# istellartech/GELATO

Hardware: NVIDIA B200
Metric: fd_jacobian_plus_residual_evals_per_s (higher is better)
Workload: dtype f64

## Files before the change

### gelato_b200/csrc/gelato_b200.cu

```cuda
#include <cuda_runtime.h>

#include <cstdio>
#include <cstdlib>
#include <cstring>
#include <string>
#include <thread>
#include <utility>
#include <vector>

#include "host_pool.h"
#include "plan_host.h"

#ifndef GJ_MIN_BLOCKS
#define GJ_MIN_BLOCKS 2
#endif
#ifndef GJ_PREFETCH_BLOCKS
#define GJ_PREFETCH_BLOCKS 296
#endif
__device__ __forceinline__ void prefetch_batch_l2(const double* x_all, size_t n_doubles, int blocks, int threads) {
#if GJ_PREFETCH_BLOCKS > 0
  if ((int)blockIdx.x < blocks) {
    const size_t lines = (n_doubles * sizeof(double) + 127) / 128;
    for (size_t l = (size_t)blockIdx.x * threads + threadIdx.x; l < lines; l += (size_t)blocks * threads)
      asm volatile("prefetch.global.L2 [%0];" ::"l"(reinterpret_cast<const char*>(x_all) + l * 128));
  }
#endif
}
#ifdef GJ_CLOCKS
__device__ unsigned long long gj_clk_sum[8][16][6];
#define GJ_CLK_DECL long long clk_[6] = {0, 0, 0, 0, 0, 0}
#define GJ_CLK(i) clk_[i] = clock64()
#define GJ_CLK_FLUSH(role, two)                                                                         \
  if ((threadIdx.x & 31) == 0) {                                                                        \
    unsigned long long* c = gj_clk_sum[(role) & 7][threadIdx.x >> 5];                                   \
    atomicAdd(c + 0, (unsigned long long)(clk_[1] - clk_[0]));                                              \
    atomicAdd(c + 1, (unsigned long long)(clk_[2] - clk_[1]));                                              \
    atomicAdd(c + 2, (unsigned long long)((two) ? 0 : clk_[3] - clk_[2]));                                  \
    atomicAdd(c + 3, (unsigned long long)((two) ? 0 : clk_[4] - clk_[3]));                                  \
    atomicAdd(c + 4, (unsigned long long)(clk_[5] - clk_[4]));                                              \
    atomicAdd(c + 5, 1ull);                                                                             \
  }
#else
#define GJ_CLK_DECL
#define GJ_CLK(i)
#define GJ_CLK_FLUSH(role, two)
#endif
template <int ROLES>
__device__ __forceinline__ void jacobian_body(const PlanView& P, const int32_t* __restrict__ block_table, const int n_scen,
                                              const int32_t* __restrict__ scen_ids, const double* __restrict__ x_all,
                                              double* __restrict__ out_all, double* __restrict__ g_all) {
  __shared__ JacStore store;
  const JacScratch sm = jac_scratch(store);
  prefetch_batch_l2(x_all, (size_t)n_scen * P.n_vars, GJ_PREFETCH_BLOCKS, GJ_THREADS);
  const int scen = blockIdx.x % n_scen;
  const int32_t* bt = block_table + (size_t)(blockIdx.x / n_scen) * BT_COLS;
  const double* x = x_all + (size_t)scen * P.n_vars;
  double* out = out_all + (size_t)scen * (size_t)(P.packed ? P.n_pack : P.n_vals);
  double* g = g_all ? g_all + (size_t)scen * P.n_rows : nullptr;
  const int sid = scen_ids ? scen_ids[scen] : scen;
  const bool two_phase = jac_role_two_phase(bt[BT_ROLE]);
  GJ_CLK_DECL;
  GJ_CLK(0);
  jac_block_phase<ROLES>(P, sid, bt, x, out, g, threadIdx.x, 0, sm);
  GJ_CLK(1);
  __syncthreads();
  GJ_CLK(2);
  if (!two_phase) {
    jac_block_phase<ROLES>(P, sid, bt, x, out, g, threadIdx.x, 2, sm);
    GJ_CLK(3);
    __syncthreads();
  }
  GJ_CLK(4);
  jac_block_phase<ROLES>(P, sid, bt, x, out, g, threadIdx.x, 3, sm);
  GJ_CLK(5);
  GJ_CLK_FLUSH(bt[BT_ROLE], two_phase);
}
__global__ void __launch_bounds__(GJ_THREADS, GJ_MIN_BLOCKS)
k_jacobian(const __grid_constant__ PlanView P, const int32_t* __restrict__ block_table, const int n_scen, const int32_t* __restrict__ scen_ids,
           const double* __restrict__ x_all, double* __restrict__ out_all, double* __restrict__ g_all) {
  jacobian_body<JR_ALL>(P, block_table, n_scen, scen_ids, x_all, out_all, g_all);
}
__global__ void __launch_bounds__(GJ_THREADS, GJ_MIN_BLOCKS)
k_jacobian_heavy(const __grid_constant__ PlanView P, const int32_t* __restrict__ block_table, const int n_scen,
                 const int32_t* __restrict__ scen_ids, const double* __restrict__ x_all, double* __restrict__ out_all,
                 double* __restrict__ g_all) {
  jacobian_body<JR_HEAVY>(P, block_table, n_scen, scen_ids, x_all, out_all, g_all);
}
__global__ void __launch_bounds__(GJ_THREADS, GJ_MIN_BLOCKS)
k_jacobian_light(const __grid_constant__ PlanView P, const int32_t* __restrict__ block_table, const int n_scen,
                 const int32_t* __restrict__ scen_ids, const double* __restrict__ x_all, double* __restrict__ out_all,
                 double* __restrict__ g_all) {
  jacobian_body<JR_LIGHT>(P, block_table, n_scen, scen_ids, x_all, out_all, g_all);
}

#define GV_THREADS (32 * GV_PARTS)
#ifndef GV_MIN_BLOCKS
#define GV_MIN_BLOCKS 5
#endif
__global__ void __launch_bounds__(GV_THREADS, GV_MIN_BLOCKS)
k_jacobian_noair(const __grid_constant__ PlanView P, const int first, const int count, const int n_scen,
                 const int32_t* __restrict__ scen_ids, const double* __restrict__ x_all, double* __restrict__ out_all,
                 double* __restrict__ g_all) {
  const int per = (count + 31) / 32;
  const int scen = blockIdx.x / per;
  const int lane = threadIdx.x & 31, part = threadIdx.x >> 5;
  const int k = (blockIdx.x - scen * per) * 32 + lane;
  __shared__ double grav[32][NPV * 3];
  const double* x = x_all + (size_t)scen * P.n_vars;
  double* out = out_all + (size_t)scen * (size_t)(P.packed ? P.n_pack : P.n_vals);
  double* g = g_all ? g_all + (size_t)scen * P.n_rows : nullptr;
  const int sid = scen_ids ? scen_ids[scen] : scen;
  const bool live = k < count;
  NodeRef nr;
  if (live) {
    nr = jac_node(P, first + k);
    for (int pv = part; pv < NPV; pv += GV_PARTS) dyn_noair_gravity(P, sid, x, nr, pv, grav[lane] + 3 * pv);
  }
  __syncthreads();
  if (live) dyn_noair_part(P, sid, x, out, g, nr, part, grav[lane]);
}

#ifndef GR_MIN_BLOCKS
#define GR_MIN_BLOCKS 8
#endif
__global__ void __launch_bounds__(GR_THREADS, GR_MIN_BLOCKS)
// ... 52 lines not shown
__global__ void k_fp64_muladd(double* out, int iters) {
  double a0 = threadIdx.x * 1e-9, a1 = a0 + 1, a2 = a0 + 2, a3 = a0 + 3, a4 = a0 + 4, a5 = a0 + 5, a6 = a0 + 6,
         a7 = a0 + 7;
  const double b = 1.0000001, c = 1e-9;
  for (int i = 0; i < iters; i++) {
    a0 = __dadd_rn(__dmul_rn(a0, b), c); a1 = __dadd_rn(__dmul_rn(a1, b), c);
    a2 = __dadd_rn(__dmul_rn(a2, b), c); a3 = __dadd_rn(__dmul_rn(a3, b), c);
    a4 = __dadd_rn(__dmul_rn(a4, b), c); a5 = __dadd_rn(__dmul_rn(a5, b), c);
    a6 = __dadd_rn(__dmul_rn(a6, b), c); a7 = __dadd_rn(__dmul_rn(a7, b), c);
  }
  out[blockIdx.x * blockDim.x + threadIdx.x] = a0 + a1 + a2 + a3 + a4 + a5 + a6 + a7;
}

static thread_local std::string g_err;
static int fail(int code, const std::string& msg) {
  g_err = msg;
  return code;
}
#define CU(call)                                                                                  \
  do {                                                                                            \
    cudaError_t e_ = (call);                                                                      \
    if (e_ != cudaSuccess)                                                                        \
      return fail(GELATO_ERR_CUDA, std::string(#call) + ": " + cudaGetErrorString(e_));           \
  } while (0)

struct GelatoPlan {
  int device = 0;
  PlanView view{};
  std::vector<void*> owned;
  int32_t* jac_blocks = nullptr;
  int n_jac_blocks = 0, n_jac_main = 0;
  int32_t *jac_heavy = nullptr, *jac_light = nullptr;
  int n_jac_heavy = 0, n_jac_light = 0;
  int vac_first = 0, n_vac = 0;
  int32_t* res_blocks = nullptr;
  int n_res_blocks = 0;
  long long n_pack = 0;
  std::vector<int64_t> pk_full, pk_src;
  std::vector<double> pk_sgn;
  std::vector<void*> scen_owned;
  double *d_packed = nullptr, *h_packed = nullptr;
  size_t cap_packed = 0;
  double *d_px = nullptr, *d_pg = nullptr, *h_px = nullptr;
  int32_t* d_pids = nullptr;
  bool pids_iota = false;
  size_t cap_px = 0;
  double* vals_template = nullptr;
  long long vals_template_sstride = 0;
  int n_scen_cfg = 1;
  cudaStream_t stream = nullptr;
  double *d_x = nullptr, *d_g = nullptr, *d_vals = nullptr;
  double *h_x = nullptr, *h_out = nullptr;
  size_t cap_scen = 0;
  cudaGraphExec_t res_graph = nullptr;
  int res_graph_n = 0;
  double* h_small_out = nullptr;
  size_t cap_small_out = 0;
  int32_t* d_ids = nullptr;
  double* d_vals_ids = nullptr;
  size_t cap_ids = 0;
  const int64_t* d_xdep = nullptr;
  std::vector<int64_t> h_xdep;
  long long n_xdep = 0;
  double *d_pack = nullptr, *h_pack = nullptr;
  size_t cap_pack = 0;
  int host_threads = 0;
// ... 26 lines not shown
  void* d = nullptr;
  CU(cudaMalloc(&d, count * sizeof(T)));
  p->owned.push_back(d);
  CU(cudaMemcpy(d, src, count * sizeof(T), cudaMemcpyHostToDevice));
  *dst = static_cast<const T*>(d);
  return GELATO_OK;
}

struct JacRange {
  int b0 = 0, nb = -1, v0 = 0, nv = 0;
};
static int launch_jacobian(GelatoPlan* p, const double* x_dev, double* out_dev, double* g_dev, int n_scen, cudaStream_t st,
                           cudaStream_t aux, cudaEvent_t ev_fork, cudaEvent_t ev_join, const int32_t* ids_dev, bool packed,
                           JacRange rg = JacRange()) {
  PlanView v = p->view;
  v.packed = packed ? 1 : 0;
  const bool all = rg.nb < 0;
  const int nb = all ? (g_dev ? p->n_jac_blocks : p->n_jac_main) : rg.nb;
  const int nv = all ? p->n_vac : rg.nv;
  const int v_first = p->vac_first + (all ? 0 : rg.v0);
  const int32_t* table = p->jac_blocks + (size_t)(all ? 0 : rg.b0) * BT_COLS;
  const bool side = nv > 0 && nb > 0 && aux != st;
  if (side) {
    CU(cudaEventRecord(ev_fork, st));
    CU(cudaStreamWaitEvent(aux, ev_fork, 0));
  }
  if (nv > 0) {
    const int per = (nv + 31) / 32;
    k_jacobian_noair<<<(unsigned)per * n_scen, GV_THREADS, 0, side ? aux : st>>>(v, v_first, nv, n_scen, ids_dev, x_dev, out_dev,
                                                                                g_dev);
    p->launches++;
  }
  if (nb > 0) {
    k_jacobian<<<(unsigned)nb * n_scen, GJ_THREADS, 0, st>>>(v, table, n_scen, ids_dev, x_dev, out_dev, g_dev);
    p->launches++;
  }
  CU(cudaGetLastError());
  if (side) {
    CU(cudaEventRecord(ev_join, aux));
    CU(cudaStreamWaitEvent(st, ev_join, 0));
  }
  return GELATO_OK;
}

extern "C" {

const char* gelato_last_error(void) { return g_err.c_str(); }
void gelato_set_error_(const char* msg) { g_err = msg ? msg : ""; }

int gelato_device_count(void) {
  int n = 0;
  if (cudaGetDeviceCount(&n) != cudaSuccess) return 0;
  return n;
}

int gelato_plan_create(const GelatoPlanDesc* d, int device, GelatoPlan** out) {
  if (!d || !out) return fail(GELATO_ERR_ARG, "null argument");
  if (const char* why = validate_desc(d)) return fail(GELATO_ERR_ARG, why);
  int ndev = 0;
  cudaError_t e = cudaGetDeviceCount(&ndev);
  if (e != cudaSuccess || ndev == 0)
    return fail(GELATO_ERR_CUDA, "no CUDA device: the B200 kernels are the only evaluation path (no CPU fallback)");
  CU(cudaSetDevice(device));
  GelatoPlan* p = new GelatoPlan();
  p->device = device;
  PlanView& v = p->view;
  planview_scalars(d, v);
// ... 25 lines not shown
    p->h_xdep.assign(d->xdep_idx, d->xdep_idx + d->n_xdep);
    p->n_xdep = d->n_xdep;
    const int64_t* dx = nullptr;
    if ((rc = upload(p, d->xdep_idx, (size_t)d->n_xdep, &dx)) != GELATO_OK) { gelato_plan_destroy(p); return rc; }
    p->d_xdep = dx;
    std::vector<int64_t> small;
    for (int64_t i = 0; i < d->n_xdep;) {
      int64_t j = i + 1;
      while (j < d->n_xdep && d->xdep_idx[j] == d->xdep_idx[j - 1] + 1) j++;
      if (j - i >= 512) p->big_runs.push_back({d->xdep_idx[i], j - i});
      else small.insert(small.end(), d->xdep_idx + i, d->xdep_idx + j);
      i = j;
    }
    p->n_small = (long long)small.size();
    p->h_small = small;
    if ((rc = upload(p, small.data(), small.size(), &dx)) != GELATO_OK) { gelato_plan_destroy(p); return rc; }
    p->d_xdep_small = dx;
  }
  const double* tmpl = nullptr;
  if ((rc = upload(p, d->vals_template, (size_t)d->n_vals, &tmpl)) != GELATO_OK) { gelato_plan_destroy(p); return rc; }
  p->vals_template = const_cast<double*>(tmpl);
#undef UP

  HostTables ht;
  build_host_tables(d, ht);
  const int32_t* tb = nullptr;
  p->n_jac_blocks = (int)(ht.jac_blocks.size() / BT_COLS);
  p->n_res_blocks = (int)(ht.res_blocks.size() / BT_COLS);
  p->n_jac_main = ht.n_jac_main;
  p->vac_first = ht.vac_first;
  p->n_vac = ht.n_vac;
  p->n_jac_heavy = (int)(ht.jac_heavy.size() / BT_COLS);
  p->n_jac_light = (int)(ht.jac_light.size() / BT_COLS);
  if ((rc = upload(p, ht.jac_heavy.data(), ht.jac_heavy.size(), &tb)) != GELATO_OK) { gelato_plan_destroy(p); return rc; }
  p->jac_heavy = const_cast<int32_t*>(tb);
  if ((rc = upload(p, ht.jac_light.data(), ht.jac_light.size(), &tb)) != GELATO_OK) { gelato_plan_destroy(p); return rc; }
  p->jac_light = const_cast<int32_t*>(tb);
  {
    PackedLayout L;
    build_packed_layout(d, L);
    if (d->xdep_idx && d->n_xdep > 0 &&
        ((size_t)d->n_xdep != L.full_slot.size() || !std::equal(L.full_slot.begin(), L.full_slot.end(), d->xdep_idx))) {
      gelato_plan_destroy(p);
      return fail(GELATO_ERR_ARG, "xdep_idx is not the set of slots the Jacobian kernel writes for this plan");
    }
    p->n_pack = L.n_pack;
    v.n_pack = L.n_pack;
    if ((rc = upload(p, L.sec_pk.data(), L.sec_pk.size(), &v.sec_pk)) != GELATO_OK) { gelato_plan_destroy(p); return rc; }
    if ((rc = upload(p, L.aero_pk.data(), L.aero_pk.size(), &v.aero_pk)) != GELATO_OK) { gelato_plan_destroy(p); return rc; }
    if ((rc = upload(p, L.evt_pk.data(), L.evt_pk.size(), &v.evt_pk)) != GELATO_OK) { gelato_plan_destroy(p); return rc; }
    p->pk_full.swap(L.full_slot);
    p->pk_src.swap(L.src);
    p->pk_sgn.swap(L.sgn);
  }
  if ((rc = upload(p, ht.jac_blocks.data(), ht.jac_blocks.size(), &tb)) != GELATO_OK) { gelato_plan_destroy(p); return rc; }
  p->jac_blocks = const_cast<int32_t*>(tb);
  if ((rc = upload(p, ht.res_blocks.data(), ht.res_blocks.size(), &tb)) != GELATO_OK) { gelato_plan_destroy(p); return rc; }
  p->res_blocks = const_cast<int32_t*>(tb);
  if ((rc = upload(p, ht.node_rec.data(), ht.node_rec.size(), &v.node_rec)) != GELATO_OK) { gelato_plan_destroy(p); return rc; }
  if ((rc = upload(p, ht.jac_rec.data(), ht.jac_rec.size(), &v.jac_rec)) != GELATO_OK) { gelato_plan_destroy(p); return rc; }
  if ((rc = upload(p, ht.aero_rows.data(), ht.aero_rows.size(), &v.aero_rows)) != GELATO_OK) { gelato_plan_destroy(p); return rc; }
  v.n_aero_rows = (int)ht.aero_rows.size();

  cudaError_t ce = cudaStreamCreateWithFlags(&p->stream, cudaStreamNonBlocking);
  if (ce == cudaSuccess) ce = cudaStreamCreateWithFlags(&p->copy_stream, cudaStreamNonBlocking);
  if (ce == cudaSuccess) ce = cudaEventCreateWithFlags(&p->ev_kernel, cudaEventDisableTiming);
// ... 739 lines not shown
    CU(cudaGetLastError());
    float ms = 0.f;
    CU(cudaEventElapsedTime(&ms, p->ev0, p->ev1));
    out_ms[piece] = ms / reps;
  }
  return GELATO_OK;
}

int gelato_host_alloc(size_t bytes, void** out) {
  if (!out) return fail(GELATO_ERR_ARG, "null");
  CU(cudaMallocHost(out, bytes));
  return GELATO_OK;
}

int gelato_host_free(void* ptr) {
  if (ptr) CU(cudaFreeHost(ptr));
  return GELATO_OK;
}

int gelato_launch_kernel_dev(GelatoPlan* p, int which, const double* x_dev, double* out_dev, double* g_dev, int32_t n_scen,
                             int32_t packed, void* stream) {
  int rc = check_scen(p, n_scen);
  if (rc) return rc;
  CU(cudaSetDevice(p->device));
  cudaStream_t st = stream ? (cudaStream_t)stream : p->stream;
  PlanView v = p->view;
  v.packed = packed ? 1 : 0;
  if (which == 0) {
    k_residuals<<<(unsigned)p->n_res_blocks * n_scen, GR_THREADS, 0, st>>>(v, p->res_blocks, n_scen, nullptr, x_dev, out_dev);
  } else if (which == 1) {
    return launch_jacobian(p, x_dev, out_dev, g_dev, n_scen, st, p->pair_stream, p->ev_fork, p->ev_join, nullptr, packed != 0);
  } else if (which == 2) {
    if (p->n_jac_heavy == 0) return fail(GELATO_ERR_ARG, "the plan has no heavy blocks");
    k_jacobian_heavy<<<(unsigned)p->n_jac_heavy * n_scen, GJ_THREADS, 0, st>>>(v, p->jac_heavy, n_scen, nullptr, x_dev, out_dev, g_dev);
  } else if (which == 3) {
    if (p->n_jac_light == 0) return fail(GELATO_ERR_ARG, "the plan has no light blocks");
    k_jacobian_light<<<(unsigned)p->n_jac_light * n_scen, GJ_THREADS, 0, st>>>(v, p->jac_light, n_scen, nullptr, x_dev, out_dev, g_dev);
  } else if (which == 5) {
    if (p->n_vac == 0) return fail(GELATO_ERR_ARG, "the plan has no vacuum nodes");
    const int per = (p->n_vac + 31) / 32;
    k_jacobian_noair<<<(unsigned)per * n_scen, GV_THREADS, 0, st>>>(v, p->vac_first, p->n_vac, n_scen, nullptr, x_dev, out_dev, g_dev);
  } else if (which == 6) {
    const int nb = g_dev ? p->n_jac_blocks : p->n_jac_main;
    if (nb == 0) return fail(GELATO_ERR_ARG, "the plan has no Jacobian blocks");
    k_jacobian<<<(unsigned)nb * n_scen, GJ_THREADS, 0, st>>>(v, p->jac_blocks, n_scen, nullptr, x_dev, out_dev, g_dev);
  } else {
    return fail(GELATO_ERR_ARG, "which must be 0, 1, 2, 3, 5 or 6");
  }
  p->launches++;
  CU(cudaGetLastError());
  return GELATO_OK;
}

int gelato_time_kernel(GelatoPlan* p, int which, const double* x_dev, double* out_dev, int32_t n_scen, int reps,
                       float* avg_ms) {
  int rc = check_scen(p, n_scen);
  if (rc) return rc;
  if (reps <= 0 || !avg_ms) return fail(GELATO_ERR_ARG, "bad reps");
  CU(cudaSetDevice(p->device));
  CU(cudaStreamSynchronize(p->stream));
  CU(cudaEventRecord(p->ev0, p->stream));
  for (int i = 0; i < reps; i++) {
    if (which == 0) {
      k_residuals<<<(unsigned)p->n_res_blocks * n_scen, GR_THREADS, 0, p->stream>>>(p->view, p->res_blocks, n_scen, nullptr, x_dev, out_dev);
    } else if (which == 1) {
      if ((rc = launch_jacobian(p, x_dev, out_dev, nullptr, n_scen, p->stream, p->pair_stream, p->ev_fork, p->ev_join, nullptr,
                                false)))
        return rc;
      continue;
    } else if (which == 2) {
      if (p->n_jac_heavy > 0)
        k_jacobian_heavy<<<(unsigned)p->n_jac_heavy * n_scen, GJ_THREADS, 0, p->stream>>>(p->view, p->jac_heavy, n_scen, nullptr,
                                                                                        x_dev, out_dev, nullptr);
    } else {
      if (p->n_jac_light > 0)
        k_jacobian_light<<<(unsigned)p->n_jac_light * n_scen, GJ_THREADS, 0, p->stream>>>(p->view, p->jac_light, n_scen, nullptr,
                                                                                        x_dev, out_dev, nullptr);
    }
    p->launches++;
  }
  CU(cudaEventRecord(p->ev1, p->stream));
  CU(cudaEventSynchronize(p->ev1));
  CU(cudaGetLastError());
  float ms = 0.f;
  CU(cudaEventElapsedTime(&ms, p->ev0, p->ev1));
  *avg_ms = ms / reps;
  return GELATO_OK;
}

int gelato_selftest_unfused(int device, int* ok) {
  if (!ok) return fail(GELATO_ERR_ARG, "null");
  CU(cudaSetDevice(device));
  double* d = nullptr;
  CU(cudaMalloc(&d, sizeof(double)));
  k_unfused_probe<<<1, 1>>>(1.0 + 0x1p-30, 1.0 - 0x1p-30, -1.0, d);
  double h = 1.0;
  CU(cudaMemcpy(&h, d, sizeof(double), cudaMemcpyDeviceToHost));
  cudaFree(d);
  *ok = (h == 0.0);
  return GELATO_OK;
}

int gelato_fp64_peak(int device, double* tflops_fma, double* tflops_nofma) {
  CU(cudaSetDevice(device));
  cudaDeviceProp prop;
  CU(cudaGetDeviceProperties(&prop, device));
  const int blocks = prop.multiProcessorCount * 8, threads = 256, iters = 1 << 14;
  double* d = nullptr;
  CU(cudaMalloc(&d, (size_t)blocks * threads * sizeof(double)));
  cudaEvent_t e0, e1;
// ... 39 lines not shown
```

### gelato_b200/csrc/jobs.h

```cpp
#ifndef GELATO_B200_JOBS_H_
#define GELATO_B200_JOBS_H_

#include "../../include/gelato_b200.h"
#include "physics.h"

#ifndef GJ_THREADS
#define GJ_THREADS 448
#endif
#ifndef GJ_NODES
#define GJ_NODES 32
#endif
#ifndef GD_NODES
#define GD_NODES 32
#endif
#ifndef GJ_A_THREADS
#define GJ_A_THREADS 160
#endif
#ifndef GJA_A_THREADS
#define GJA_A_THREADS 192
#endif
#ifndef GD_GRAVITY_IN_POS
#define GD_GRAVITY_IN_POS 0
#endif
#ifndef GN_NODES
// ... 3 lines not shown
#define GN_A_THREADS 160
#endif
#ifndef GJ_EVT_PER_WARP
#define GJ_EVT_PER_WARP 0
#endif
#ifndef GJ_EVT
#define GJ_EVT (GJ_THREADS / (GJ_EVT_PER_WARP ? 32 : 16))
#endif
#ifndef GG_NODES
#define GG_NODES (GJ_THREADS / 16)
#endif
#define GR_THREADS 128
#define GR_NODES 64
#define NPV 5
#define NRV 7
#define NPVA 6
#define NRVA 8
#define NQV 8

static_assert(GJ_A_THREADS % 32 == 0 && GJ_A_THREADS < GJ_THREADS && GJ_THREADS % 32 == 0, "phase-0 thread groups are whole warps");
static_assert(GJA_A_THREADS % 32 == 0 && GJA_A_THREADS < GJ_THREADS, "phase-0 thread groups are whole warps");
static_assert(GN_A_THREADS % 32 == 0 && GN_A_THREADS < GJ_THREADS, "no-air thread groups are whole warps");
static_assert(GG_NODES * 16 <= GJ_THREADS && GJ_EVT * 16 <= GJ_THREADS, "lane maps");
#define GJ_MAX2(a, b) ((a) > (b) ? (a) : (b))
#define GJ_FQ_NODES GJ_MAX2(GJ_MAX2(GN_NODES, GD_NODES), GG_NODES)
#define GJ_PR_NODES GJ_MAX2(GJ_NODES, GD_NODES)
static_assert(GJ_THREADS * 3 <= GJ_FQ_NODES * 14 * 3, "event jobs keep 3 values per thread in f");
static_assert(GN_NODES * NPV * 3 <= GJ_PR_NODES * NPVA * 8, "no-air gravity items fit the pp array");
static_assert(GR_THREADS == 2 * GR_NODES, "residual phase 0 uses two threads per node");

enum { BR_DYN_AIR = 0, BR_DYN_NOAIR, BR_DYN_GEN, BR_AERO, BR_EVT, BR_LIN, BR_DYN  };
enum { BT_ROLE = 0, BT_JOB, BT_START, BT_COUNT, BT_COLS };
#define GJ_PHASES 4

struct PlanView {
  int S, N, M, n_vars, n_rows;
  long long n_vals;
  int payload_mode;
  int off_pos, off_vel, off_quat, off_u, off_t;
  const int32_t* sec_i32;
  const int64_t* sec_i64;
  const double* sec_f64;
  long long sec_f64_sstride;
  const double* d_pool;
  const double* tau_pool;
  const double* wind;
  long long wind_sstride;
  int n_wind;
  const double* ca;
  int n_ca;
  Units un;
  const double* unit_mass_scen;
  int n_lin;
  const int32_t* lin_i32;
  const double* lin_f64;
  const double* lin_const_scen;
  int n_aero;
  const int32_t* aero_i32;
  const int64_t* aero_i64;
  const double* aero_f64;
  const uint8_t* rc_aero;
  int n_evt;
  const int32_t* evt_i32;
  const int64_t* evt_i64;
  const double* evt_f64;
  const struct NodeRec* node_rec;
// ... 959 lines not shown
    return;
  }
  if (type == GE_USER_ORBIT) {
    for (int r = 0; r < ei[GE_NROW]; r++)
      vals[ej[GE_J_POS] + r * GE_USER_AUX + (lane - 1)] = fd_div(sm.f[3 * tid + r] - sm.f[3 * c + r], dx);
    return;
  }
  const int comp = ei[GE_COMP], form = ei[GE_FORM];
  const double gfd = fd_div(sm.f[3 * tid + comp] - sm.f[3 * c + comp], dx);
  const double val = evt_form_grad(form, gfd, ef[GE_REF], ef[GE_DEN]);
  if (type == GE_IIP) {
    if (lane == 7) vals[ej[GE_J_T]] = val;
    else if (lane & 1) vals[ej[GE_J_POS] + (lane - 1) / 2] = val;
    else vals[ej[GE_J_VEL] + (lane - 2) / 2] = val;
  } else {
    if (lane == 4) vals[ej[GE_J_T]] = val;
    else vals[ej[GE_J_POS] + (lane - 1)] = val;
  }
}

P_HD void lin_res(const PlanView& P, int scen, const double* x, double* g, int k) {
  const int32_t* li = P.lin_i32 + k * GL_I32_COLS;
  const double* lf = P.lin_f64 + k * GL_F64_COLS;
  const double a = (li[GL_IDX_PLUS] >= 0) ? x[li[GL_IDX_PLUS]] * lf[GL_SCALE_PLUS] : 0.0;
  const double b = (li[GL_IDX_MINUS] >= 0) ? x[li[GL_IDX_MINUS]] * lf[GL_SCALE_MINUS] : 0.0;
  const double c = P.lin_const_scen ? P.lin_const_scen[(long long)scen * P.n_lin + k] : lf[GL_CONST];
  g[li[GL_ROW]] = (a - b) + c;
}

#define JR_HEAVY ((1 << BR_DYN_AIR) | (1 << BR_AERO))
#define JR_LIGHT ((1 << BR_DYN_NOAIR) | (1 << BR_DYN_GEN) | (1 << BR_EVT) | (1 << BR_LIN))
#define JR_ALL (JR_HEAVY | JR_LIGHT)
P_HD void lin_res(const PlanView& P, int scen, const double* x, double* g, int k);
template <int ROLES>
GM_HD_INL void jac_block_phase(const PlanView& P, int scen, const int32_t* bt, const double* x, double* vals, double* g,
                          int tid, int phase, const JacScratch& sm) {
  const int start = bt[BT_START], count = bt[BT_COUNT], role = bt[BT_ROLE];
  if ((ROLES >> BR_DYN_AIR & 1) && role == BR_DYN_AIR) dyn_air_phase(P, scen, x, vals, g, start, count, tid, phase, sm);
  if ((ROLES >> BR_AERO & 1) && role == BR_AERO) aero_phase(P, scen, x, vals, g, start, count, tid, phase, sm);
  if ((ROLES >> BR_DYN_NOAIR & 1) && role == BR_DYN_NOAIR) dyn_noair_phase(P, scen, x, vals, g, start, count, tid, phase, sm);
  if ((ROLES >> BR_DYN_GEN & 1) && role == BR_DYN_GEN) dyn_gen_phase(P, scen, x, vals, g, start, count, tid, phase, sm);
  if ((ROLES >> BR_EVT & 1) && role == BR_EVT && (tid >> (GJ_EVT_PER_WARP ? 5 : 4)) < count &&
      (!GJ_EVT_PER_WARP || (tid & 31) < 16)) {
    const int job = tid >> (GJ_EVT_PER_WARP ? 5 : 4);
    const int slot = job * 16 + (tid & (GJ_EVT_PER_WARP ? 31 : 15));
    if (phase == 0) evt_jac_phase1(P, scen, x, start + job, slot, g != nullptr, sm);
    else if (phase == 3) evt_jac_phase2(P, vals, g, start + job, slot, sm);
  }
  if ((ROLES >> BR_LIN & 1) && role == BR_LIN && phase == 3 && g) {
    if (tid < count) lin_res(P, scen, x, g, start + tid);
    if (start == 0 && tid == 0) g[0] = P.payload_mode ? -x[0] : x[P.off_t + P.S];
  }
}
P_HD bool jac_role_two_phase(int role) { return role == BR_EVT || role == BR_DYN_GEN || role == BR_LIN; }

P_HD void res_block_phase0(const PlanView& P, int scen, const int32_t* bt, const double* x, int tid, ResScratch& sm) {
  if (bt[BT_ROLE] == BR_DYN) dyn_res_phase0(P, scen, x, bt[BT_START], bt[BT_COUNT], tid, sm);
}
P_HD void res_block_phase1(const PlanView& P, int scen, const int32_t* bt, const double* x, double* g, int tid,
                           ResScratch& sm) {
  switch (bt[BT_ROLE]) {
    case BR_DYN: dyn_res_phase1(P, scen, x, bt[BT_START], bt[BT_COUNT], tid, sm); break;
    case BR_AERO:
      if (tid < bt[BT_COUNT]) {
        aero_res(P, scen, x, g, P.aero_rows[bt[BT_START] + tid]);
      }
      break;
    case BR_EVT:
      if (tid < bt[BT_COUNT]) evt_res(P, scen, x, g, bt[BT_START] + tid);
      break;
    case BR_LIN:
      if (tid < bt[BT_COUNT]) lin_res(P, scen, x, g, bt[BT_START] + tid);
      if (bt[BT_START] == 0 && tid == 0)
        g[0] = P.payload_mode ? -x[0] : x[P.off_t + P.S];
      break;
    default: break;
  }
}
P_HD void res_block_phase2(const PlanView& P, int scen, const int32_t* bt, const double* x, double* g, int tid,
                           int nthreads, const ResScratch& sm) {
  if (bt[BT_ROLE] == BR_DYN) dyn_res_phase2(P, scen, x, g, bt[BT_START], bt[BT_COUNT], tid, nthreads, sm);
}

#endif
```

### gelato_b200/csrc/plan_host.h

```cpp
#ifndef GELATO_B200_PLAN_HOST_H_
#define GELATO_B200_PLAN_HOST_H_

#include <algorithm>
#include <vector>

#include "jobs.h"

static inline void planview_scalars(const GelatoPlanDesc* d, PlanView& v) {
  const int S = d->n_sections, N = d->n_nodes, M = N + S;
  v.S = S; v.N = N; v.M = M;
  v.n_vars = M + 3 * M + 3 * M + 4 * M + 2 * N + S + 1;
  v.n_rows = d->n_rows;
  v.n_vals = d->n_vals;
  v.payload_mode = d->payload_mode;
  v.off_pos = M; v.off_vel = 4 * M; v.off_quat = 7 * M; v.off_u = 11 * M; v.off_t = 11 * M + 2 * N;
  v.un.mass = d->unit_mass; v.un.pos = d->unit_pos; v.un.vel = d->unit_vel; v.un.u = d->unit_u;
  v.un.t = d->unit_t; v.un.dx = d->dx;
  v.n_wind = d->n_wind; v.n_ca = d->n_ca;
  v.n_lin = d->n_lin; v.n_aero = d->n_aero; v.n_evt = d->n_evt;
}

static inline const char* validate_desc(const GelatoPlanDesc* d) {
  if (!d) return "null description";
  const long long S = d->n_sections, N = d->n_nodes, M = N + S;
// ... 59 lines not shown
    if (!GELATO_RANGE(sj[GS_JP_VEL], 3 * n) || !GELATO_RANGE(sj[GS_JP_T], 6 * n) || !GELATO_RANGE(sj[GS_JV_MASS], 3 * n) ||
        !GELATO_RANGE(sj[GS_JV_POS], 9 * n) || !GELATO_RANGE(sj[GS_JV_QUAT], 12 * n) || !GELATO_RANGE(sj[GS_JV_T], 6 * n))
      return "a section's Jacobian block offset is outside vals";
    if ((fl & GSF_AIR_FD) && !GELATO_RANGE(sj[GS_JV_VEL], 9 * n * (n + 1))) return "a section's velocity block is outside vals";
    if (!(fl & GSF_HOLD) && (!GELATO_RANGE(sj[GS_JQ_QUAT], 16 * n * (n + 1)) || !GELATO_RANGE(sj[GS_JQ_U], 8 * n) ||
                             !GELATO_RANGE(sj[GS_JQ_T], 8 * n)))
      return "a section's quaternion block is outside vals";
  }
  for (long long k = 0; k < d->n_aero; k++) {
    const int32_t* ai = d->aero_i32 + k * GA_I32_COLS;
    const int64_t* aj = d->aero_i64 + k * GA_I64_COLS;
    const long long nk = ai[GA_NK];
    if (!GELATO_RANGE(aj[GA_J_POS], 3 * nk) || !GELATO_RANGE(aj[GA_J_VEL], 3 * nk) || !GELATO_RANGE(aj[GA_J_T], 2 * nk) ||
        (ai[GA_KIND] != 1 && !GELATO_RANGE(aj[GA_J_QUAT], 4 * nk)))
      return "an aero job's Jacobian block is outside vals";
  }
  for (long long k = 0; k < d->n_evt; k++) {
    const int32_t* ei = d->evt_i32 + k * GE_I32_COLS;
    const int64_t* ej = d->evt_i64 + k * GE_I64_COLS;
    const int type = ei[GE_TYPE];
    bool ok;
    if (type == GE_TERM) ok = GELATO_RANGE(ej[GE_J_POS], 3 * ei[GE_NROW]) && GELATO_RANGE(ej[GE_J_VEL], 3 * ei[GE_NROW]);
    else if (type >= GE_USER_ORBIT) ok = GELATO_RANGE(ej[GE_J_POS], GE_USER_AUX * ei[GE_NROW]);
    else ok = GELATO_RANGE(ej[GE_J_POS], 3) && GELATO_RANGE(ej[GE_J_T], 1) && (type != GE_IIP || GELATO_RANGE(ej[GE_J_VEL], 3));
    if (!ok) return "an event job's Jacobian block is outside vals";
  }
#undef GELATO_RANGE
  return nullptr;
}

struct HostTables {
  std::vector<int32_t> jac_blocks, jac_heavy, jac_light, res_blocks;
  int n_jac_main = 0;
  int vac_first = 0, n_vac = 0;
  std::vector<NodeRec> node_rec;
  std::vector<NodeRec> jac_rec;
  std::vector<AeroRec> aero_rows;
};

struct PackedLayout {
  std::vector<int64_t> sec_pk, aero_pk, evt_pk;
  long long n_pack = 0;
  std::vector<int64_t> full_slot, src;
  std::vector<double> sgn;
};

static inline void build_packed_layout(const GelatoPlanDesc* d, PackedLayout& L) {
  const int S = d->n_sections;
  L.sec_pk.assign((size_t)S * GS_I64_COLS, -1);
  L.aero_pk.assign((size_t)d->n_aero * GA_I64_COLS, -1);
  L.evt_pk.assign((size_t)d->n_evt * GE_I64_COLS, -1);
  struct Ent { int64_t full, src; double sgn; };
  std::vector<Ent> ents;
  long long c = 0;
  auto direct = [&](int64_t full0, long long len) {
    const long long at = c;
    for (long long i = 0; i < len; i++) ents.push_back({full0 + i, at + i, 1.0});
    c += len;
    return at;
  };
  auto mirrored = [&](int64_t full0, long long half) {
    const long long at = c;
    for (long long i = 0; i < half; i++) {
      ents.push_back({full0 + i, at + i, 1.0});
      ents.push_back({full0 + half + i, at + i, -1.0});
    }
// ... 100 lines not shown
  for (const std::vector<int32_t>* list : {&air, &vac, &gen})
    for (int32_t g : *list) h.jac_rec.push_back(h.node_rec[g]);
  for (int k = 0; k < d->n_aero; k++) {
    const int32_t* ai = d->aero_i32 + k * GA_I32_COLS;
    const int32_t* si = d->sec_i32 + ai[GA_SECTION] * GS_I32_COLS;
    for (int r = 0; r < ai[GA_NK]; r++) {
      AeroRec q;
      q.job = k; q.r = r; q.sec = ai[GA_SECTION]; q.row = si[GS_XA] + r;
      q.kind = ai[GA_KIND]; q.nk = ai[GA_NK]; q.tau_off = si[GS_TAU_OFF]; q.row0 = ai[GA_ROW0];
      h.aero_rows.push_back(q);
    }
  }
  const int n_aero_rows = (int)h.aero_rows.size();

  std::vector<int32_t> heavy, light;
  push_chunks(heavy, BR_DYN_AIR, 0, (int)air.size(), GD_NODES);
  push_chunks(heavy, BR_AERO, 0, n_aero_rows, GJ_NODES);
  push_chunks(light, BR_DYN_GEN, (int)(air.size() + vac.size()), (int)gen.size(), GG_NODES);
  push_chunks(light, BR_EVT, 0, d->n_evt, GJ_EVT);
  h.jac_heavy = heavy;
  h.jac_light = light;
  h.vac_first = (int)air.size();
  h.n_vac = (int)vac.size();
  std::vector<int32_t>& jb = h.jac_blocks;
  const long long nh = (long long)heavy.size() / BT_COLS, nl = (long long)light.size() / BT_COLS;
  for (long long ih = 0, il = 0; ih < nh || il < nl;) {
    const bool take_heavy = il >= nl || (ih < nh && ih * nl <= il * nh);
    const std::vector<int32_t>& src = take_heavy ? heavy : light;
    const long long k = take_heavy ? ih++ : il++;
    jb.insert(jb.end(), src.begin() + k * BT_COLS, src.begin() + (k + 1) * BT_COLS);
  }
  h.n_jac_main = (int)(jb.size() / BT_COLS);
  push_chunks(jb, BR_LIN, 0, d->n_lin, GJ_THREADS);

  std::vector<int32_t>& rb = h.res_blocks;
  push_chunks(rb, BR_DYN, 0, N, GR_NODES);
  push_chunks(rb, BR_AERO, 0, n_aero_rows, GR_THREADS);
  push_chunks(rb, BR_EVT, 0, d->n_evt, GR_THREADS);
  push_chunks(rb, BR_LIN, 0, d->n_lin, GR_THREADS);
}

#endif
```

Measured before the change: 10.50 billion.

## Pack multiple scenarios' event jobs into one Jacobian block

When the event job count is small, a single event block now serves several scenarios (evt_group = GJ_EVT / n_evt) rather than one per scenario. A JacGrid mapping replaces the flat blockIdx-to-(row, scenario) split, so the event row launches fewer blocks and the grid shrinks. The goal is to stop launching many mostly idle event blocks. The cost is extra index arithmetic in every block and a more complex grid mapping.

```diff
diff --git a/gelato_b200/csrc/gelato_b200.cu b/gelato_b200/csrc/gelato_b200.cu
--- a/gelato_b200/csrc/gelato_b200.cu
+++ b/gelato_b200/csrc/gelato_b200.cu
@@ -46,51 +46,51 @@
 #define GJ_CLK_FLUSH(role, two)
 #endif
 template <int ROLES>
-__device__ __forceinline__ void jacobian_body(const PlanView& P, const int32_t* __restrict__ block_table, const int n_scen,
+__device__ __forceinline__ void jacobian_body(const PlanView& P, const int32_t* __restrict__ block_table, const JacGrid& grid,
                                               const int32_t* __restrict__ scen_ids, const double* __restrict__ x_all,
                                               double* __restrict__ out_all, double* __restrict__ g_all) {
   __shared__ JacStore store;
   const JacScratch sm = jac_scratch(store);
-  prefetch_batch_l2(x_all, (size_t)n_scen * P.n_vars, GJ_PREFETCH_BLOCKS, GJ_THREADS);
-  const int scen = blockIdx.x % n_scen;
-  const int32_t* bt = block_table + (size_t)(blockIdx.x / n_scen) * BT_COLS;
-  const double* x = x_all + (size_t)scen * P.n_vars;
-  double* out = out_all + (size_t)scen * (size_t)(P.packed ? P.n_pack : P.n_vals);
-  double* g = g_all ? g_all + (size_t)scen * P.n_rows : nullptr;
-  const int sid = scen_ids ? scen_ids[scen] : scen;
+  prefetch_batch_l2(x_all, (size_t)grid.n_scen * P.n_vars, GJ_PREFETCH_BLOCKS, GJ_THREADS);
+  int scen, n_here;
+  const int32_t* bt = block_table + (size_t)jac_grid_block(grid, blockIdx.x, &scen, &n_here) * BT_COLS;
+  JacBatch B;
+  B.x_all = x_all; B.out_all = out_all; B.g_all = g_all; B.scen_ids = scen_ids;
+  const JacSlot s = jac_slot(P, B, scen);
   const bool two_phase = jac_role_two_phase(bt[BT_ROLE]);
   GJ_CLK_DECL;
   GJ_CLK(0);
-  jac_block_phase<ROLES>(P, sid, bt, x, out, g, threadIdx.x, 0, sm);
+  jac_block_phase<ROLES>(P, B, s, bt, scen, n_here, threadIdx.x, 0, sm);
   GJ_CLK(1);
   __syncthreads();
   GJ_CLK(2);
   if (!two_phase) {
-    jac_block_phase<ROLES>(P, sid, bt, x, out, g, threadIdx.x, 2, sm);
+    jac_block_phase<ROLES>(P, B, s, bt, scen, n_here, threadIdx.x, 2, sm);
     GJ_CLK(3);
     __syncthreads();
   }
   GJ_CLK(4);
-  jac_block_phase<ROLES>(P, sid, bt, x, out, g, threadIdx.x, 3, sm);
+  jac_block_phase<ROLES>(P, B, s, bt, scen, n_here, threadIdx.x, 3, sm);
   GJ_CLK(5);
   GJ_CLK_FLUSH(bt[BT_ROLE], two_phase);
 }
 __global__ void __launch_bounds__(GJ_THREADS, GJ_MIN_BLOCKS)
-k_jacobian(const __grid_constant__ PlanView P, const int32_t* __restrict__ block_table, const int n_scen, const int32_t* __restrict__ scen_ids,
-           const double* __restrict__ x_all, double* __restrict__ out_all, double* __restrict__ g_all) {
-  jacobian_body<JR_ALL>(P, block_table, n_scen, scen_ids, x_all, out_all, g_all);
+k_jacobian(const __grid_constant__ PlanView P, const int32_t* __restrict__ block_table, const JacGrid grid,
+           const int32_t* __restrict__ scen_ids, const double* __restrict__ x_all, double* __restrict__ out_all,
+           double* __restrict__ g_all) {
+  jacobian_body<JR_ALL>(P, block_table, grid, scen_ids, x_all, out_all, g_all);
 }
 __global__ void __launch_bounds__(GJ_THREADS, GJ_MIN_BLOCKS)
-k_jacobian_heavy(const __grid_constant__ PlanView P, const int32_t* __restrict__ block_table, const int n_scen,
+k_jacobian_heavy(const __grid_constant__ PlanView P, const int32_t* __restrict__ block_table, const JacGrid grid,
                  const int32_t* __restrict__ scen_ids, const double* __restrict__ x_all, double* __restrict__ out_all,
                  double* __restrict__ g_all) {
-  jacobian_body<JR_HEAVY>(P, block_table, n_scen, scen_ids, x_all, out_all, g_all);
+  jacobian_body<JR_HEAVY>(P, block_table, grid, scen_ids, x_all, out_all, g_all);
 }
 __global__ void __launch_bounds__(GJ_THREADS, GJ_MIN_BLOCKS)
-k_jacobian_light(const __grid_constant__ PlanView P, const int32_t* __restrict__ block_table, const int n_scen,
+k_jacobian_light(const __grid_constant__ PlanView P, const int32_t* __restrict__ block_table, const JacGrid grid,
                  const int32_t* __restrict__ scen_ids, const double* __restrict__ x_all, double* __restrict__ out_all,
                  double* __restrict__ g_all) {
-  jacobian_body<JR_LIGHT>(P, block_table, n_scen, scen_ids, x_all, out_all, g_all);
+  jacobian_body<JR_LIGHT>(P, block_table, grid, scen_ids, x_all, out_all, g_all);
 }
 
 #define GV_THREADS (32 * GV_PARTS)
@@ -209,6 +209,7 @@
   int n_jac_blocks = 0, n_jac_main = 0;
   int32_t *jac_heavy = nullptr, *jac_light = nullptr;
   int n_jac_heavy = 0, n_jac_light = 0;
+  int evt_row = -1, evt_row_light = -1, evt_group = 1;
   int vac_first = 0, n_vac = 0;
   int32_t* res_blocks = nullptr;
   int n_res_blocks = 0;
@@ -301,7 +302,8 @@
     p->launches++;
   }
   if (nb > 0) {
-    k_jacobian<<<(unsigned)nb * n_scen, GJ_THREADS, 0, st>>>(v, table, n_scen, ids_dev, x_dev, out_dev, g_dev);
+    const JacGrid grid = jac_grid(n_scen, p->evt_row, p->evt_group, all ? 0 : rg.b0, nb);
+    k_jacobian<<<(unsigned)jac_grid_blocks(grid, nb), GJ_THREADS, 0, st>>>(v, table, grid, ids_dev, x_dev, out_dev, g_dev);
     p->launches++;
   }
   CU(cudaGetLastError());
@@ -393,6 +395,9 @@
   p->n_vac = ht.n_vac;
   p->n_jac_heavy = (int)(ht.jac_heavy.size() / BT_COLS);
   p->n_jac_light = (int)(ht.jac_light.size() / BT_COLS);
+  p->evt_row = ht.evt_row;
+  p->evt_row_light = ht.evt_row_light;
+  p->evt_group = ht.evt_group;
   if ((rc = upload(p, ht.jac_heavy.data(), ht.jac_heavy.size(), &tb)) != GELATO_OK) { gelato_plan_destroy(p); return rc; }
   p->jac_heavy = const_cast<int32_t*>(tb);
   if ((rc = upload(p, ht.jac_light.data(), ht.jac_light.size(), &tb)) != GELATO_OK) { gelato_plan_destroy(p); return rc; }
@@ -1198,10 +1203,14 @@
     return launch_jacobian(p, x_dev, out_dev, g_dev, n_scen, st, p->pair_stream, p->ev_fork, p->ev_join, nullptr, packed != 0);
   } else if (which == 2) {
     if (p->n_jac_heavy == 0) return fail(GELATO_ERR_ARG, "the plan has no heavy blocks");
-    k_jacobian_heavy<<<(unsigned)p->n_jac_heavy * n_scen, GJ_THREADS, 0, st>>>(v, p->jac_heavy, n_scen, nullptr, x_dev, out_dev, g_dev);
+    const JacGrid grid = jac_grid(n_scen, -1, 1, 0, p->n_jac_heavy);
+    k_jacobian_heavy<<<(unsigned)jac_grid_blocks(grid, p->n_jac_heavy), GJ_THREADS, 0, st>>>(v, p->jac_heavy, grid, nullptr, x_dev,
+                                                                                          out_dev, g_dev);
   } else if (which == 3) {
     if (p->n_jac_light == 0) return fail(GELATO_ERR_ARG, "the plan has no light blocks");
-    k_jacobian_light<<<(unsigned)p->n_jac_light * n_scen, GJ_THREADS, 0, st>>>(v, p->jac_light, n_scen, nullptr, x_dev, out_dev, g_dev);
+    const JacGrid grid = jac_grid(n_scen, p->evt_row_light, p->evt_group, 0, p->n_jac_light);
+    k_jacobian_light<<<(unsigned)jac_grid_blocks(grid, p->n_jac_light), GJ_THREADS, 0, st>>>(v, p->jac_light, grid, nullptr, x_dev,
+                                                                                          out_dev, g_dev);
   } else if (which == 5) {
     if (p->n_vac == 0) return fail(GELATO_ERR_ARG, "the plan has no vacuum nodes");
     const int per = (p->n_vac + 31) / 32;
@@ -1209,7 +1218,8 @@
   } else if (which == 6) {
     const int nb = g_dev ? p->n_jac_blocks : p->n_jac_main;
     if (nb == 0) return fail(GELATO_ERR_ARG, "the plan has no Jacobian blocks");
-    k_jacobian<<<(unsigned)nb * n_scen, GJ_THREADS, 0, st>>>(v, p->jac_blocks, n_scen, nullptr, x_dev, out_dev, g_dev);
+    const JacGrid grid = jac_grid(n_scen, p->evt_row, p->evt_group, 0, nb);
+    k_jacobian<<<(unsigned)jac_grid_blocks(grid, nb), GJ_THREADS, 0, st>>>(v, p->jac_blocks, grid, nullptr, x_dev, out_dev, g_dev);
   } else {
     return fail(GELATO_ERR_ARG, "which must be 0, 1, 2, 3, 5 or 6");
   }
@@ -1235,13 +1245,15 @@
         return rc;
       continue;
     } else if (which == 2) {
+      const JacGrid grid = jac_grid(n_scen, -1, 1, 0, p->n_jac_heavy);
       if (p->n_jac_heavy > 0)
-        k_jacobian_heavy<<<(unsigned)p->n_jac_heavy * n_scen, GJ_THREADS, 0, p->stream>>>(p->view, p->jac_heavy, n_scen, nullptr,
-                                                                                        x_dev, out_dev, nullptr);
+        k_jacobian_heavy<<<(unsigned)jac_grid_blocks(grid, p->n_jac_heavy), GJ_THREADS, 0, p->stream>>>(p->view, p->jac_heavy, grid,
+                                                                                                      nullptr, x_dev, out_dev, nullptr);
     } else {
+      const JacGrid grid = jac_grid(n_scen, p->evt_row_light, p->evt_group, 0, p->n_jac_light);
       if (p->n_jac_light > 0)
-        k_jacobian_light<<<(unsigned)p->n_jac_light * n_scen, GJ_THREADS, 0, p->stream>>>(p->view, p->jac_light, n_scen, nullptr,
-                                                                                        x_dev, out_dev, nullptr);
+        k_jacobian_light<<<(unsigned)jac_grid_blocks(grid, p->n_jac_light), GJ_THREADS, 0, p->stream>>>(p->view, p->jac_light, grid,
+                                                                                                      nullptr, x_dev, out_dev, nullptr);
     }
     p->launches++;
   }
diff --git a/gelato_b200/csrc/jobs.h b/gelato_b200/csrc/jobs.h
--- a/gelato_b200/csrc/jobs.h
+++ b/gelato_b200/csrc/jobs.h
@@ -59,6 +59,38 @@
 enum { BR_DYN_AIR = 0, BR_DYN_NOAIR, BR_DYN_GEN, BR_AERO, BR_EVT, BR_LIN, BR_DYN  };
 enum { BT_ROLE = 0, BT_JOB, BT_START, BT_COUNT, BT_COLS };
 #define GJ_PHASES 4
+
+struct JacGrid {
+  int n_scen, evt_row, evt_group;
+};
+P_HD int jac_grid_blocks(const JacGrid& G, int n_rows) {
+  const int short_by = G.evt_row < n_rows ? G.n_scen - (G.n_scen + G.evt_group - 1) / G.evt_group : 0;
+  return n_rows * G.n_scen - short_by;
+}
+P_HD int jac_grid_block(const JacGrid& G, int b, int* scen, int* n_here) {
+  const int e0 = G.evt_row * G.n_scen;
+  *n_here = 1;
+  if (b >= e0) {
+    const int ne = (G.n_scen + G.evt_group - 1) / G.evt_group;
+    if (b < e0 + ne) {
+      *scen = (b - e0) * G.evt_group;
+      *n_here = G.n_scen - *scen < G.evt_group ? G.n_scen - *scen : G.evt_group;
+      return G.evt_row;
+    }
+    b += G.n_scen - ne;
+  }
+  const int row = b / G.n_scen;
+  *scen = b - row * G.n_scen;
+  return row;
+}
+P_HD JacGrid jac_grid(int n_scen, int evt_row, int evt_group, int b0, int nb) {
+  const bool has = evt_row >= b0 && evt_row < b0 + nb;
+  JacGrid G;
+  G.n_scen = n_scen;
+  G.evt_row = has ? evt_row - b0 : nb;
+  G.evt_group = has ? evt_group : 1;
+  return G;
+}
 
 struct PlanView {
   int S, N, M, n_vars, n_rows;
@@ -1084,25 +1116,59 @@
 #define JR_LIGHT ((1 << BR_DYN_NOAIR) | (1 << BR_DYN_GEN) | (1 << BR_EVT) | (1 << BR_LIN))
 #define JR_ALL (JR_HEAVY | JR_LIGHT)
 P_HD void lin_res(const PlanView& P, int scen, const double* x, double* g, int k);
+struct JacBatch {
+  const double* x_all;
+  double* out_all;
+  double* g_all;
+  const int32_t* scen_ids;
+};
+struct JacSlot {
+  const double* x;
+  double* out;
+  double* g;
+  int sid;
+};
+P_HD JacSlot jac_slot(const PlanView& P, const JacBatch& B, int scen) {
+  JacSlot s;
+  s.x = B.x_all + (size_t)scen * P.n_vars;
+  s.out = B.out_all + (size_t)scen * (size_t)(P.packed ? P.n_pack : P.n_vals);
+  s.g = B.g_all ? B.g_all + (size_t)scen * P.n_rows : nullptr;
+  s.sid = B.scen_ids ? B.scen_ids[scen] : scen;
+  return s;
+}
 template <int ROLES>
-GM_HD_INL void jac_block_phase(const PlanView& P, int scen, const int32_t* bt, const double* x, double* vals, double* g,
-                          int tid, int phase, const JacScratch& sm) {
+GM_HD_INL void jac_block_phase(const PlanView& P, const JacBatch& B, const JacSlot& s, const int32_t* bt, int scen, int n_here,
+                               int tid, int phase, const JacScratch& sm) {
   const int start = bt[BT_START], count = bt[BT_COUNT], role = bt[BT_ROLE];
-  if ((ROLES >> BR_DYN_AIR & 1) && role == BR_DYN_AIR) dyn_air_phase(P, scen, x, vals, g, start, count, tid, phase, sm);
-  if ((ROLES >> BR_AERO & 1) && role == BR_AERO) aero_phase(P, scen, x, vals, g, start, count, tid, phase, sm);
-  if ((ROLES >> BR_DYN_NOAIR & 1) && role == BR_DYN_NOAIR) dyn_noair_phase(P, scen, x, vals, g, start, count, tid, phase, sm);
-  if ((ROLES >> BR_DYN_GEN & 1) && role == BR_DYN_GEN) dyn_gen_phase(P, scen, x, vals, g, start, count, tid, phase, sm);
-  if ((ROLES >> BR_EVT & 1) && role == BR_EVT && (tid >> (GJ_EVT_PER_WARP ? 5 : 4)) < count &&
-      (!GJ_EVT_PER_WARP || (tid & 31) < 16)) {
-    const int job = tid >> (GJ_EVT_PER_WARP ? 5 : 4);
-    const int slot = job * 16 + (tid & (GJ_EVT_PER_WARP ? 31 : 15));
-    if (phase == 0) evt_jac_phase1(P, scen, x, start + job, slot, g != nullptr, sm);
-    else if (phase == 3) evt_jac_phase2(P, vals, g, start + job, slot, sm);
+  const double* x = s.x;
+  double* const vals = s.out;
+  double* const g = s.g;
+  if ((ROLES >> BR_DYN_AIR & 1) && role == BR_DYN_AIR) dyn_air_phase(P, s.sid, x, vals, g, start, count, tid, phase, sm);
+  if ((ROLES >> BR_AERO & 1) && role == BR_AERO) aero_phase(P, s.sid, x, vals, g, start, count, tid, phase, sm);
+  if ((ROLES >> BR_DYN_NOAIR & 1) && role == BR_DYN_NOAIR) dyn_noair_phase(P, s.sid, x, vals, g, start, count, tid, phase, sm);
+  if ((ROLES >> BR_DYN_GEN & 1) && role == BR_DYN_GEN) dyn_gen_phase(P, s.sid, x, vals, g, start, count, tid, phase, sm);
+  if ((ROLES >> BR_EVT & 1) && role == BR_EVT && (!GJ_EVT_PER_WARP || (tid & 31) < 16)) {
+    const int js = tid >> (GJ_EVT_PER_WARP ? 5 : 4);
+    const int k = js / count;
+    if (k < n_here) {
+      const int job = js - k * count;
+      const int slot = js * 16 + (tid & (GJ_EVT_PER_WARP ? 31 : 15));
+      const JacSlot e = jac_slot(P, B, scen + k);
+      if (phase == 0) evt_jac_phase1(P, e.sid, e.x, start + job, slot, e.g != nullptr, sm);
+      else if (phase == 3) evt_jac_phase2(P, e.out, e.g, start + job, slot, sm);
+    }
   }
   if ((ROLES >> BR_LIN & 1) && role == BR_LIN && phase == 3 && g) {
-    if (tid < count) lin_res(P, scen, x, g, start + tid);
+    if (tid < count) lin_res(P, s.sid, x, g, start + tid);
     if (start == 0 && tid == 0) g[0] = P.payload_mode ? -x[0] : x[P.off_t + P.S];
   }
+}
+template <int ROLES>
+GM_HD_INL void jac_block_phase(const PlanView& P, int sid, const int32_t* bt, const double* x, double* vals, double* g,
+                               int tid, int phase, const JacScratch& sm) {
+  JacBatch B;
+  B.x_all = x; B.out_all = vals; B.g_all = g; B.scen_ids = &sid;
+  jac_block_phase<ROLES>(P, B, jac_slot(P, B, 0), bt, 0, 1, tid, phase, sm);
 }
 P_HD bool jac_role_two_phase(int role) { return role == BR_EVT || role == BR_DYN_GEN || role == BR_LIN; }
 
diff --git a/gelato_b200/csrc/plan_host.h b/gelato_b200/csrc/plan_host.h
--- a/gelato_b200/csrc/plan_host.h
+++ b/gelato_b200/csrc/plan_host.h
@@ -115,6 +115,7 @@
 struct HostTables {
   std::vector<int32_t> jac_blocks, jac_heavy, jac_light, res_blocks;
   int n_jac_main = 0;
+  int evt_row = -1, evt_row_light = -1, evt_group = 1;
   int vac_first = 0, n_vac = 0;
   std::vector<NodeRec> node_rec;
   std::vector<NodeRec> jac_rec;
@@ -281,6 +282,12 @@
   }
   h.n_jac_main = (int)(jb.size() / BT_COLS);
   push_chunks(jb, BR_LIN, 0, d->n_lin, GJ_THREADS);
+  if (d->n_evt > 0 && d->n_evt <= GJ_EVT) {
+    h.evt_group = GJ_EVT / d->n_evt;
+    for (int b = 0; b < h.n_jac_main; b++)
+      if (jb[(size_t)b * BT_COLS + BT_ROLE] == BR_EVT) h.evt_row = b;
+    h.evt_row_light = (int)(light.size() / BT_COLS) - 1;
+  }
 
   std::vector<int32_t>& rb = h.res_blocks;
   push_chunks(rb, BR_DYN, 0, N, GR_NODES);
```

Result: faster. 10.93 billion (median of 6 runs) (+4.1%).
